# Hanbo-Cheng/DAWN-pytorch

Measured on NVIDIA H100. Metric: denoising-steps/sec (200-frame 256^2 clip), higher is better.
Workload: dtype f32

## Files before the change

dawn_pytorch_b200/_lib.py:

```python
import ctypes
import os

import torch

_HERE = os.path.dirname(os.path.abspath(__file__))
LIB_PATH = os.path.join(_HERE, "libdawn_unet.so")


class DawnUnetCfg(ctypes.Structure):
    _fields_ = [("dim", ctypes.c_int), ("n_levels", ctypes.c_int), ("dim_mults", ctypes.c_int * 8),
                ("channels", ctypes.c_int), ("cond_aud", ctypes.c_int), ("cond_pose", ctypes.c_int),
                ("cond_eye", ctypes.c_int), ("out_grid_dim", ctypes.c_int), ("out_conf_dim", ctypes.c_int),
                ("attn_heads", ctypes.c_int), ("attn_dim_head", ctypes.c_int), ("resnet_groups", ctypes.c_int),
                ("init_kernel_size", ctypes.c_int), ("win_width", ctypes.c_int),
                ("upconv", ctypes.c_int), ("pad_mode", ctypes.c_int), ("no_sla", ctypes.c_int)]


class DawnLfgCfg(ctypes.Structure):
    _fields_ = [("num_channels", ctypes.c_int), ("block_expansion", ctypes.c_int), ("max_features", ctypes.c_int),
                ("num_down_blocks", ctypes.c_int), ("num_bottleneck_blocks", ctypes.c_int), ("skips", ctypes.c_int)]


PATH_MMA_SYNC, PATH_TC_GEMM, PATH_TC_GEMM_PRESPLIT, PATH_TC_CONV3, PATH_TC_CONV3_TMA = range(5)
EPI_PLAIN, EPI_QKV_TEMPORAL, EPI_QKV_SLA, EPI_QKV_MID, EPI_CA_GATE, EPI_GN_APPLY = range(6)


class DawnContractionCase(ctypes.Structure):
    _i, _p = ctypes.c_int, ctypes.c_void_p
    _fields_ = [("path", _i), ("epi", _i),
                ("F", _i), ("IH", _i), ("IW", _i), ("Cin", _i), ("lda", _i),
                ("ntaps", _i), ("dy", _i * 52), ("dx", _i * 52), ("in_stride", _i),
                ("OHs", _i), ("OWs", _i), ("OH", _i), ("OW", _i), ("out_stride", _i), ("oy0", _i), ("ox0", _i),
                ("up2", _i),
                ("perm_pb", _i), ("perm_F", _i), ("perm_in", _i), ("perm_out", _i), ("perm_f_lo", _i), ("perm_f_hi", _i),
                ("P", _i),
                ("N", _i), ("ldb", _i), ("ldo", _i), ("ldr", _i), ("drain", _i), ("ln_inline", _i),
                ("rows_per_batch", _i), ("b_batch_stride", ctypes.c_longlong), ("cpg", _i),
                ("q_post_scale", ctypes.c_float),
                ("A", _p), ("B", _p), ("bias", _p), ("Res", _p), ("Out", _p),
                ("stats", _p), ("rowstats", _p), ("wsum", _p), ("rot", _p),
                ("kq", _p), ("nkq", _p), ("gates", _p),
                ("Y", _p), ("ldy", _i), ("gn_stats", _p), ("gn_w", _p), ("gn_b", _p), ("film", _p), ("gn_count", ctypes.c_double)]


FUSED_TEMPORAL, FUSED_ATTN_TC, FUSED_ATTN_SIMT, FUSED_SLA_CTX, FUSED_SLA_OUT, FUSED_SLA_CTX_UNFUSED, FUSED_CA_WT, \
    FUSED_CA_RSTD, FUSED_GN_HCOND, FUSED_TEMPORAL_MMA_SYNC = range(10)


class DawnFusedCase(ctypes.Structure):
    _i, _p = ctypes.c_int, ctypes.c_void_p
    _fields_ = [("kernel", _i), ("F", _i), ("P", _i), ("C", _i), ("band", _i), ("q_lo", _i), ("q_hi", _i),
                ("nseq", _i), ("L", _i), ("pb", _i), ("seq_base_stride", ctypes.c_longlong), ("elem_stride", ctypes.c_longlong),
                ("ldx", _i), ("ldr", _i), ("ldo", _i), ("ld", _i), ("ldb", _i), ("ldy", _i), ("ldbT", _i),
                ("x", _p), ("res", _p), ("out", _p), ("gamma", _p), ("w_qkv", _p), ("w_out", _p), ("rot", _p), ("bias", _p),
                ("qkv", _p), ("Bf", _p), ("out_bias", _p), ("kq", _p), ("nkq", _p), ("G", _p), ("gates", _p), ("Wt", _p),
                ("T", _p), ("Y", _p), ("out16h", _p), ("out16l", _p),
                ("gn_stats", _p), ("gn_count", ctypes.c_double), ("cpg", _i), ("gn_w", _p), ("gn_b", _p), ("film", _p)]


KERNEL_ROWSTATS, KERNEL_GN_APPLY, KERNEL_COND_TABLES, KERNEL_TIME_MLP, KERNEL_FILM, KERNEL_ROTARY, KERNEL_SPLIT_ROWS, \
    KERNEL_NCF_TO_NHWC, KERNEL_FRAME_INVARIANCE, KERNEL_FEA_SHIFT, KERNEL_MAP_REDUCE, KERNEL_INIT_CONV_X3, KERNEL_HEADS_OUT, \
    KERNEL_DDIM_STEP, KERNEL_DDPM_STEP = range(15)
KERNEL_MAX_DESC = 16


class DawnKernelDesc(ctypes.Structure):
    _i, _p = ctypes.c_int, ctypes.c_void_p
    _fields_ = [("off", _i), ("K", _i), ("co", _i), ("ldbT", _i), ("ca", _i),
                ("mW", _p), ("mB", _p), ("Wkv", _p), ("nkv", _p), ("qs", _p), ("ks", _p), ("Wout", _p), ("gout", _p),
                ("ctx", _p), ("kv", _p), ("kq", _p), ("nkq", _p), ("T", _p), ("G", _p),
                ("W", _p), ("b", _p), ("out", _p), ("n", _i)]


class DawnKernelCase(ctypes.Structure):
    _i, _p, _ll = ctypes.c_int, ctypes.c_void_p, ctypes.c_longlong
    _fields_ = [("kernel", _i), ("M", _i), ("C", _i), ("ld", _i), ("ldy", _i), ("ldr", _i), ("ldo", _i),
                ("F", _i), ("H", _i), ("W", _i), ("P", _i), ("clips", _i),
                ("Cpad", _i), ("c0", _i), ("k", _i), ("skip_if", _i), ("cpg", _i), ("t_stride", _i), ("pos0", _i), ("dim", _i),
                ("ng", _i), ("nc", _i), ("cond_ld", _i), ("ndesc", _i),
                ("n", _ll), ("cstride", _ll), ("clip_stride", _ll), ("count", ctypes.c_double), ("eps", ctypes.c_float),
                ("x", _p), ("y", _p), ("res", _p), ("w", _p), ("b", _p), ("w2", _p), ("b2", _p),
                ("map", _p), ("freqs", _p), ("stats", _p), ("t", _p), ("skip_flag", _p),
                ("out", _p), ("out_hi", _p), ("out_lo", _p), ("flag", _p),
                ("desc", DawnKernelDesc * KERNEL_MAX_DESC),
                ("xs", _p), ("e", _p), ("noise", _p), ("scratch", _p), ("tab", _p), ("t_slot", _p), ("num_t", _i),
                ("replicas", _i), ("coef", ctypes.c_float * 5), ("q", ctypes.c_float)]


LFG_MOTION_PACK, LFG_WARP_BLEND, LFG_AFFINE_RELU, LFG_RESIDUAL_BN_RELU, LFG_RELU_AVGPOOL2, LFG_CHW_TO_HWC, LFG_HWC_TO_CHW, \
    LFG_FINAL_CONV = range(8)


class DawnLfgKernelCase(ctypes.Structure):
    _i, _p = ctypes.c_int, ctypes.c_void_p
    _fields_ = [("kernel", _i), ("F", _i), ("H", _i), ("W", _i), ("h", _i), ("w", _i), ("C", _i), ("Cpad", _i),
# ... 188 lines not shown
```

dawn_pytorch_b200/csrc/contraction.cu:

```cuda
#include <algorithm>
#include <cmath>
#include <cstring>

#include "common.cuh"
#include "contraction.cuh"
#include "kernels.cuh"
#include "tc_gemm.cuh"

namespace dawn {

void HostParams::set(const std::string& name, const float* data, const int64_t* shape, int ndim) {
  HostParam p;
  p.shape.assign(shape, shape + ndim);
  int64_t numel = 1;
  for (int64_t s : p.shape) numel *= s;
  p.data.assign(data, data + numel);
  map[name] = std::move(p);
}

int HostParams::need(const std::string& name, const std::vector<int64_t>& shape, const HostParam** out) const {
  auto it = map.find(name);
  if (it == map.end()) { set_last_error(prefix + "missing parameter: " + name); return -1; }
  const HostParam& p = it->second;
  if (p.shape != shape) {
// ... 234 lines not shown
}

int pack_lfg_up(const HostParams& raw, std::vector<void*>& owner, const std::string& name, int co, int ci, UpConv* u) {
  const HostParam *w, *b;
  DAWN_TRY(raw.need(name + ".conv.weight", {co, ci, 3, 3}, &w));
  DAWN_TRY(raw.need(name + ".conv.bias", {co}, &b));
  std::vector<double> s, t;
  DAWN_TRY(bn_affine(raw, name + ".norm", co, s, t));
  std::vector<float> bias(co);
  for (int n = 0; n < co; ++n) bias[n] = (float)((double)b->data[n] * s[n] + t[n]);
  return pack_up_nearest(owner, w->data.data(), ci, co, s.data(), bias, u);
}

int run_up(const GemmParams& in, const UpConv& u, float* out, int ldo, const std::function<int(const GemmParams&)>& run, int border) {
  if (!border) {
    GemmParams p = in;
    set_weights(p, u.all); set_square_taps(p, 3, 1);
    p.up2 = 1; p.Out = out; p.ldo = ldo;
    if (path_ok(p, EPI_PLAIN, DAWN_PATH_TC_CONV3, 0)) return run(p);
  }
  for (int py = 0; py < 2; ++py)
    for (int px = 0; px < 2; ++px) {
      GemmParams q = in;
      set_weights(q, u.cls[py * 2 + px]);
      q.ntaps = 4;
      for (int ty = 0; ty < 2; ++ty)
        for (int tx = 0; tx < 2; ++tx) {
          q.dy[ty * 2 + tx] = (signed char)(u.off[py][ty] + border); q.dx[ty * 2 + tx] = (signed char)(u.off[px][tx] + border);
        }
      q.OH = 2 * in.OHs; q.OW = 2 * in.OWs; q.out_stride = 2; q.oy0 = py; q.ox0 = px;
      q.Out = out; q.ldo = ldo;
      DAWN_TRY(run(q));
    }
  return 0;
}

namespace {

int refuse(const char* why) {
  set_last_error(std::string("dawn_test_contraction: ") + why);
  return -1;
}

struct Owned {
  std::vector<void*> v;
  ~Owned() { free_all(v); }
};

int test_contraction(const dawn_contraction_case& c, cudaStream_t st) {
  if (c.path < DAWN_PATH_MMA_SYNC || c.path > DAWN_PATH_TC_CONV3_TMA) return refuse("unknown path");
  if (c.epi < EPI_PLAIN || c.epi > EPI_GN_APPLY) return refuse("unknown epilogue");
  if (c.ntaps < 1 || c.ntaps > 52 || c.F < 1 || c.N < 1 || c.ldb < c.N || c.lda < c.Cin) return refuse("bad geometry");
  if (!c.A || !c.B) return refuse("A and B are required");
  if (c.epi == EPI_CA_GATE ? !c.gates : !c.Out) return refuse("no output buffer");

  GemmParams p;
  memset(&p, 0, sizeof(p));
  p.A = c.A; p.lda = c.lda; p.Cin = c.Cin;
  p.up2 = c.up2;
  p.IH = c.IH; p.IW = c.IW; p.OHs = c.OHs; p.OWs = c.OWs; p.in_stride = c.in_stride;
  p.ntaps = c.ntaps;
  for (int t = 0; t < c.ntaps; ++t) { p.dy[t] = (signed char)c.dy[t]; p.dx[t] = (signed char)c.dx[t]; }
  p.M = c.F * c.OHs * c.OWs; p.N = c.N; p.K = c.ntaps * c.Cin;
  p.rows_per_batch = c.rows_per_batch > 0 ? c.rows_per_batch : p.M;
  p.perm_pb = c.perm_pb; p.perm_F = c.perm_F; p.perm_in = c.perm_in; p.perm_out = c.perm_out;
  p.perm_f_lo = c.perm_f_lo; p.perm_f_hi = c.perm_f_hi;
  p.B = c.B; p.ldb = c.ldb; p.b_batch_stride = c.b_batch_stride;
  p.Out = c.Out; p.ldo = c.ldo; p.OH = c.OH; p.OW = c.OW; p.out_stride = c.out_stride; p.oy0 = c.oy0; p.ox0 = c.ox0;
  p.bias = c.bias; p.Res = c.Res; p.ldr = c.ldr;
  p.stats = c.stats; p.cpg = c.cpg; p.clips = 1;
  p.rowstats = c.rowstats; p.ln_inline = c.ln_inline; p.wsum = c.wsum; p.rot = c.rot; p.P = c.P;
  p.q_post_scale = c.q_post_scale;
  p.kq = c.kq; p.nkq = c.nkq; p.gates = c.gates;
  p.Y = c.Y; p.ldy = c.ldy; p.gn_stats = c.gn_stats; p.gn_w = c.gn_w; p.gn_b = c.gn_b; p.film = c.film; p.gn_count = c.gn_count;
  p.drain = c.drain;

  const bool ln = c.epi >= EPI_QKV_TEMPORAL && c.epi <= EPI_CA_GATE;
  if (p.ln_inline && (c.path != DAWN_PATH_TC_GEMM || p.ntaps != 1)) return refuse("inline LayerNorm statistics need the gather-producer wgmma GEMM and one tap");
  if (ln && !p.ln_inline && !p.rowstats) return refuse("LayerNorm epilogue without row statistics");
  if (ln && !p.wsum) return refuse("LayerNorm epilogue without wsum");
  if (c.epi == EPI_PLAIN && p.stats && (p.cpg <= 0 || p.N / p.cpg > 8)) return refuse("GroupNorm statistics need 8 groups");

  Owned own;
  if (c.path != DAWN_PATH_MMA_SYNC) {
    std::vector<float> hB((size_t)p.K * p.ldb);
    DAWN_CUDA_OK(cudaMemcpy(hB.data(), p.B, hB.size() * sizeof(float), cudaMemcpyDeviceToHost));
    PackedWeight w;
    DAWN_TRY(upload_weight(own.v, hB, p.K, p.N, p.ldb, {}, &w));
    set_weights(p, w);
    p.bias = c.bias;
  }
  const bool split = c.path == DAWN_PATH_TC_GEMM_PRESPLIT || c.path == DAWN_PATH_TC_CONV3_TMA;
  const size_t scratch_bytes = split ? (size_t)split_rows(p) * p.Cin * 4 : 0;
  if (!path_ok(p, c.epi, c.path, scratch_bytes)) return refuse("the path does not accept this geometry");
  float* scratch = nullptr;
  if (split) DAWN_TRY(dev_alloc(own.v, scratch_bytes / sizeof(float), &scratch));
  DAWN_TRY(launch_path(p, c.epi, c.path, scratch, st));
  DAWN_CUDA_OK(cudaStreamSynchronize(st));
  return 0;
}

}
}

extern "C" int dawn_test_contraction(const dawn_contraction_case* c, void* stream) {
  if (!c) return dawn::refuse("null case");
  return dawn::test_contraction(*c, static_cast<cudaStream_t>(stream));
}
```

dawn_pytorch_b200/csrc/gemm.cuh:

```cuda
#pragma once
#include <cuda_runtime.h>

namespace dawn {

enum Epi : int {
  EPI_PLAIN = 0,
  EPI_QKV_TEMPORAL = 1,
  EPI_QKV_SLA = 2,
  EPI_QKV_MID = 3,
  EPI_CA_GATE = 4,
  EPI_GN_APPLY = 5,
};

struct GemmParams {
  const float* A; int lda; int Cin;
  const unsigned short* A16h = nullptr; const unsigned short* A16l = nullptr;
  int want_split = 0;
  int up2 = 0;
  int IH, IW;
  int OHs, OWs;
  int in_stride;
  int ntaps; signed char dy[52]; signed char dx[52];
  int M, N, K;
  int rows_per_batch;
  int perm_pb, perm_F, perm_in, perm_out;
  int perm_f_lo, perm_f_hi;
  const float* B; int ldb; long long b_batch_stride;
  const float* Bimg;
  float tc_scale;
  float* Out; int ldo; int OH, OW, out_stride, oy0, ox0;
  const float* bias;
  const float* Res; int ldr;
  double* stats; int cpg;
  int clips;
  const float* rowstats;
  int ln_inline;
  const float* wsum;
  const float* rot;
  int P;
  float q_post_scale;
  const float* kq;
  const float* nkq;
  float* gates;
  const float* Y; int ldy; const double* gn_stats; const float* gn_w; const float* gn_b;
  const float* film;
  double gn_count;
  const int* skip_flag; int skip_if;
  int drain;
};

__host__ __device__ inline int seq_blocked_pixel(int m, int pb, int F, int P) {
  const int blk = m / (F * pb), rem = m - blk * F * pb;
  const int f = rem / pb, pi = rem - f * pb;
  return f * P + blk * pb + pi;
}
__host__ __device__ inline int seq_blocked_out_pixel(int m, int pb, int F, int P, int f_lo, int f_hi) {
  const int blk = m / (F * pb), rem = m - blk * F * pb;
  const int f = rem / pb, pi = rem - f * pb;
  if (f < f_lo || f >= f_hi) return -1;
  return (f - f_lo) * P + blk * pb + pi;
}

int launch_gemm(const GemmParams& p, int epi, cudaStream_t st);

}
```

dawn_pytorch_b200/csrc/tc_conv3.cu:

```cuda
#include <cuda.h>
#include <cuda_fp16.h>
#include <cstdlib>
#include <cstring>
#include <string>
#include <map>
#include <tuple>
#include "common.cuh"
#include "f16x3.cuh"
#include "gemm.cuh"
#include "tc_common.cuh"
#include "tc_gemm.cuh"

namespace dawn {
namespace {

using namespace tc;

constexpr int TH = 16, TW = 8;
constexpr int HH = TH + 2, HW = TW + 2;
constexpr int NPROD = 256;
constexpr int PAIR_HH = 8 + 2;
constexpr int PAIR_ROW_B = 104;

template <int BN, bool PAIR = false>
struct CCfg {
  static_assert(!PAIR || BN == 64, "the pair-mode halos fit next to 64-column weight stages only");
  static constexpr int NWG = BN / 64;
  static constexpr bool SPLIT_EPI = (BN == 64);
  static constexpr int B_PANEL = BN * 128;
  static constexpr int FRAME_ROWS = PAIR ? PAIR_HH * HW : HH * HW;
  static constexpr int HALO_ROWS = PAIR ? PAIR_ROW_B + FRAME_ROWS : FRAME_ROWS;
  static constexpr int A_HALO = (HALO_ROWS * 128 + 1023) / 1024 * 1024;
  static constexpr int A_STAGES = 2;
  static constexpr int B_STAGES = PAIR ? 3 : (BN == 64) ? 4 : 2;
  static constexpr int A_BYTES = A_STAGES * 2 * A_HALO;
  static constexpr int B_BYTES = B_STAGES * 2 * B_PANEL;
  static constexpr int ACC_STAGE = 2 * 128 * kStageLd * 4;
  static constexpr int SMEM_DYN = A_BYTES + B_BYTES + ACC_STAGE + 1024;
  static_assert(SMEM_DYN + 1024 <= 232448, "shared memory");
  static constexpr int EPI_WARP = NPROD / 32 + 4 * NWG;
  static constexpr int LOAD_WARP = EPI_WARP + (SPLIT_EPI ? 4 : 0);
  static constexpr int NTHREADS = 32 * LOAD_WARP + 128;
  static constexpr uint32_t REG_LAUNCH = (65536 / NTHREADS) & ~7u;
  static constexpr uint32_t REG_LOAD = 24, REG_MMA = SPLIT_EPI ? 136 : 128, REG_EPI = 128;
  static_assert(REG_LOAD < REG_LAUNCH && REG_MMA > REG_LAUNCH && REG_EPI > REG_LAUNCH, "register budgets");
  static_assert(2 * REG_LAUNCH + REG_LOAD + NWG * REG_MMA + (SPLIT_EPI ? REG_EPI : 0) <= NTHREADS / 128 * REG_LAUNCH, "CTA register pool");
};

template <int BN, bool TMA, bool PAIR>
__device__ __forceinline__ void tc_conv3_body(const GemmParams& p, const float* __restrict__ Bimg, int tiles_y, int tiles_x, int tiles_n,
                                              int img_bn, const CUtensorMap& tm_hi, const CUtensorMap& tm_lo) {
  using C = CCfg<BN, PAIR>;
  constexpr int B_PANEL = C::B_PANEL, A_STAGES = C::A_STAGES, B_STAGES = C::B_STAGES, NWG = C::NWG;
  constexpr int A_HALO = C::A_HALO, FRAME_ROWS = C::FRAME_ROWS;
  constexpr bool SPLIT = C::SPLIT_EPI;
  extern __shared__ uint8_t smem_raw[];
  __shared__ uint64_t a_full[A_STAGES], a_free[A_STAGES], b_full[B_STAGES], b_free[B_STAGES];
  __shared__ uint64_t st_full[2], st_free[2];
  __shared__ float s_stat[NWG][16];
  __shared__ __align__(16) float s_bias[NWG][64];

  const int tid = threadIdx.x, lane = tid & 31;
  const int warp = __shfl_sync(0xffffffffu, tid >> 5, 0);
  uint8_t* smem = smem_align1024(smem_raw);
  uint8_t* smemA = smem;
  uint8_t* smemB = smem + C::A_BYTES;
  float* stage_base = reinterpret_cast<float*>(smemB + C::B_BYTES);

  if (tid == 0) {
    for (int s = 0; s < A_STAGES; ++s) { mbar_init(&a_full[s], TMA ? 1 : NPROD); mbar_init(&a_free[s], 4 * NWG); }
    for (int s = 0; s < B_STAGES; ++s) { mbar_init(&b_full[s], 1); mbar_init(&b_free[s], 4 * NWG); }
    for (int s = 0; s < 2; ++s) { mbar_init(&st_full[s], 128); mbar_init(&st_free[s], 128); }
    asm volatile("fence.mbarrier_init.release.cluster;" ::: "memory");
  }
  __syncthreads();

  const int H = p.IH, W = p.IW;
  const int F = p.M / (H * W);
  const int NCH = p.Cin / 64;
  const int tiles_sp = tiles_y * tiles_x;
  const int fpc = F / p.clips;
  const int ppc = (fpc + 1) / 2;
  const int total_tiles = (PAIR ? p.clips * ppc : F * tiles_sp) * tiles_n;
  auto decode = [&](int tile, int& f, int& y0, int& x0, int& nt, int& nf) {
    nt = tile % tiles_n;
    const int sp = tile / tiles_n;
    if constexpr (PAIR) {
      const int clip = sp / ppc, fa = 2 * (sp - clip * ppc);
      f = fa * p.clips + clip;
      nf = fa + 1 < fpc ? 2 : 1;
      y0 = 0; x0 = 0;
    } else {
      const int seq = sp / tiles_sp;
      const int r = sp - seq * tiles_sp;
      f = p.clips == 1 ? seq : (seq % fpc) * p.clips + seq / fpc;
      nf = 1;
      y0 = (r / tiles_x) * TH; x0 = (r % tiles_x) * TW;
    }
  };

  if (warp < 8) {
    if (TMA) {
      if (tid == 0) {
        const uint64_t mh = reinterpret_cast<uint64_t>(&tm_hi), ml = reinterpret_cast<uint64_t>(&tm_lo);
        uint32_t ait = 0;
        for (int tile = blockIdx.x; tile < total_tiles; tile += gridDim.x) {
          int f, y0, x0, nt, nf;
          decode(tile, f, y0, x0, nt, nf);
          for (int cc = 0; cc < NCH; ++cc, ++ait) {
            const int s = ait % A_STAGES;
            mbar_wait(&a_free[s], ((ait / A_STAGES) & 1) ^ 1);
            mbar_arrive_expect_tx(&a_full[s], nf * 2 * FRAME_ROWS * 128);
// ... 26 lines not shown
          auto load = [&](int q, float4& a, float4& b) {
            const int l = r0 + 32 * q;
            const int fr = (!PAIR || 32 * q + 31 < FRAME_ROWS) ? 0 : (32 * q >= FRAME_ROWS) ? 1 : (l >= FRAME_ROWS ? 1 : 0);
            const int r = l - fr * FRAME_ROWS;
            const int hy = r / HW, hx = r - hy * HW;
            const int iy = y0 + hy - 1, ix = x0 + hx - 1;
            const bool ok = (r < FRAME_ROWS) && fr < nf && (iy >= 0) && (iy < H) && (ix >= 0) && (ix < W);
            if (ok) {
              const float* fimg = fr ? img_b : img;
              const float4* src = reinterpret_cast<const float4*>(fimg + (size_t)(iy * W + ix) * p.lda + cc * 64) + 2 * c16;
              a = __ldg(src);
              b = __ldg(src + 1);
            } else {
              a = make_float4(0.f, 0.f, 0.f, 0.f);
              b = make_float4(0.f, 0.f, 0.f, 0.f);
            }
          };
          uint8_t* a_hi = smemA + s * 2 * A_HALO;
          uint8_t* a_lo = a_hi + A_HALO;
          auto store = [&](int q, const float4& a, const float4& b) {
            const int lr = r0 + 32 * q;
            const int fr = (!PAIR || 32 * q + 31 < FRAME_ROWS) ? 0 : (32 * q >= FRAME_ROWS) ? 1 : (lr >= FRAME_ROWS ? 1 : 0);
            const int r = lr + fr * (PAIR_ROW_B - FRAME_ROWS);
            if (lr < FRAME_ROWS * (PAIR ? 2 : 1)) {
              uint32_t h[4], l[4];
              split_f16x2_rn(a.x, a.y, h[0], l[0]);
              split_f16x2_rn(a.z, a.w, h[1], l[1]);
              split_f16x2_rn(b.x, b.y, h[2], l[2]);
              split_f16x2_rn(b.z, b.w, h[3], l[3]);
              const uint32_t off = swz(r, c16);
              *reinterpret_cast<uint4*>(a_hi + off) = make_uint4(h[0], h[1], h[2], h[3]);
              *reinterpret_cast<uint4*>(a_lo + off) = make_uint4(l[0], l[1], l[2], l[3]);
            }
          };
          constexpr int NPRE = NQ < 6 ? NQ : 6;
          float4 v[2 * NPRE];
#pragma unroll
          for (int q = 0; q < NPRE; ++q) load(q, v[2 * q], v[2 * q + 1]);
          mbar_wait(&a_free[s], (round & 1) ^ 1);
#pragma unroll
          for (int q = 0; q < NPRE; ++q) store(q, v[2 * q], v[2 * q + 1]);
#pragma unroll
          for (int q = NPRE; q < NQ; ++q) {
            float4 a, b;
            load(q, a, b);
            store(q, a, b);
          }
          mbar_arrive_relaxed(&a_full[s]);
        }
      }
    }
    return;
  }
  if (warp >= C::LOAD_WARP) {
    setmaxnreg_dec<C::REG_LOAD>();
    if (warp == C::LOAD_WARP && lane == 0) {
      uint32_t bit = 0;
      const int KC = 9 * NCH;
      const int sub = PAIR ? img_bn / BN : 1;
      const size_t ipanel = (size_t)sub * B_PANEL;
      for (int tile = blockIdx.x; tile < total_tiles; tile += gridDim.x) {
        int f, y0, x0, nt, nf;
        decode(tile, f, y0, x0, nt, nf);
        const uint8_t* src = reinterpret_cast<const uint8_t*>(Bimg) + (size_t)(nt / sub) * KC * (2 * ipanel) + (size_t)(nt % sub) * B_PANEL;
        for (int cc = 0; cc < NCH; ++cc)
          for (int tap = 0; tap < 9; ++tap, ++bit) {
            const int s = bit % B_STAGES;
            const uint32_t round = bit / B_STAGES;
            mbar_wait(&b_free[s], (round & 1) ^ 1);
            mbar_arrive_expect_tx(&b_full[s], 2 * B_PANEL);
            const uint8_t* panel = src + (size_t)(tap * NCH + cc) * (2 * ipanel);
            if (PAIR) {
              bulk_copy_g2s(smemB + s * 2 * B_PANEL, panel, B_PANEL, &b_full[s]);
              bulk_copy_g2s(smemB + s * 2 * B_PANEL + B_PANEL, panel + ipanel, B_PANEL, &b_full[s]);
            } else {
              bulk_copy_g2s(smemB + s * 2 * B_PANEL, panel, 2 * B_PANEL, &b_full[s]);
            }
          }
      }
    }
    return;
  }

  const int wg = SPLIT ? 0 : (warp - 8) >> 2;
  const int ew = (warp - 8) & 3;
  const int etid = ew * 32 + lane;
  const int bar_id = 2 + wg;
  constexpr uint32_t SBO_HALO = HW * 128;
  constexpr uint32_t H2 = PAIR ? PAIR_ROW_B * 128 : 8 * HW * 128;
  const int dt = (p.drain == 1 || p.drain == 3) ? p.drain : 9;

  auto mma_tile = [&](auto DTc, float* stage, uint32_t& ait, uint32_t& bit, auto&& claim) {
    constexpr int DT = decltype(DTc)::value;
    float d0[32], d1[32];
    bool first_drain = true;
    for (int cc = 0; cc < NCH; ++cc, ++ait) {
      const int sa = ait % A_STAGES;
      mbar_wait(&a_full[sa], (ait / A_STAGES) & 1);
      fence_proxy_async();
      const uint32_t a_hi = smem_u32(smemA + sa * 2 * A_HALO), a_lo = a_hi + A_HALO;
      static_for<0, 9>([&](auto TAPc) {
        constexpr int tap = decltype(TAPc)::value;
        constexpr bool group_first = tap % DT == 0, group_last = tap % DT == DT - 1;
        constexpr uint32_t woff = (uint32_t)(((tap / 3) * HW + tap % 3) * 128);
        const int sb = bit % B_STAGES;
        const int sprev = (bit + B_STAGES - 1) % B_STAGES;
        mbar_wait(&b_full[sb], (bit / B_STAGES) & 1);
        const uint64_t ahi = make_desc(a_hi + woff, SBO_HALO), alo = make_desc(a_lo + woff, SBO_HALO);
        const uint64_t ahi2 = make_desc(a_hi + woff + H2, SBO_HALO), alo2 = make_desc(a_lo + woff + H2, SBO_HALO);
        const uint32_t sbaddr = smem_u32(smemB + sb * 2 * B_PANEL) + wg * 64 * 128;
        const uint64_t bhi = make_desc(sbaddr), blo = make_desc(sbaddr + B_PANEL);
        wgmma_fence();
#pragma unroll
        for (int j = 0; j < 4; ++j) {
          const uint64_t o = (uint64_t)(j * 2);
          const uint32_t acc = (group_first && j == 0) ? 0u : 1u;
          wgmma_m64n64k16(d0, alo + o, bhi + o, acc);
          wgmma_m64n64k16(d1, alo2 + o, bhi + o, acc);
          wgmma_m64n64k16(d0, ahi + o, blo + o, 1u);
          wgmma_m64n64k16(d1, ahi2 + o, blo + o, 1u);
          wgmma_m64n64k16(d0, ahi + o, bhi + o, 1u);
          wgmma_m64n64k16(d1, ahi2 + o, bhi + o, 1u);
        }
        wgmma_commit();
        if constexpr (group_last) {
          wgmma_wait<0>();
          wgmma_fence_acc(d0); wgmma_fence_acc(d1);
          if (lane == 0) { if (!group_first) mbar_arrive(&b_free[sprev]); mbar_arrive(&b_free[sb]); }
          if (first_drain) claim();
          stage_fragment(stage, 0, d0, first_drain, etid);
          stage_fragment(stage, 64, d1, first_drain, etid);
          first_drain = false;
        } else {
          wgmma_wait<1>();
          wgmma_fence_acc(d0); wgmma_fence_acc(d1);
          if (lane == 0 && !group_first) mbar_arrive(&b_free[sprev]);
        }
        ++bit;
      });
      if (lane == 0) mbar_arrive(&a_free[sa]);
    }
  };

  const bool defer_stats = (p.stats != nullptr) && tiles_n == 1;
  const bool bias_smem = (p.bias != nullptr) && tiles_n == 1;
  auto load_bias = [&]() {
    if (bias_smem) {
      if (etid < 64) s_bias[wg][etid] = __ldg(p.bias + wg * 64 + etid);
      asm volatile("bar.sync %0, 128;" ::"r"(bar_id) : "memory");
    }
  };
  auto flush_stats = [&](float (&gs)[8], float (&gss)[8], int clip) {
    const int n0f = wg * 64;
    double* cs = p.stats + 16 * clip;
#pragma unroll
    for (int b8 = 0; b8 < 8; ++b8) {
      double s = (double)gs[b8], ss = (double)gss[b8];
#pragma unroll
      for (int o = 16; o > 0; o >>= 1) { s += __shfl_xor_sync(0xffffffffu, s, o); ss += __shfl_xor_sync(0xffffffffu, ss, o); }
      if (lane == 0) {
        const int grp = (n0f + b8 * 8) / p.cpg;
        atomicAdd(&cs[2 * grp], s);
        atomicAdd(&cs[2 * grp + 1], ss);
      }
      gs[b8] = 0.f; gss[b8] = 0.f;
    }
  };
  auto epilogue_tile = [&](int tile, float* stage, float (&gs)[8], float (&gss)[8], int& pending, int& pclip) {
    int f, y0, x0, nt, nf;
    decode(tile, f, y0, x0, nt, nf);
    const int clip = p.clips > 1 ? f % p.clips : 0;
    const int n0 = nt * BN + wg * 64;
    const int row_in_tile = etid;
    float* s_st = s_stat[wg];
    float* wbuf = stage + ew * 32 * kStageLd;
    float acc[64];
    {
      const float4* src = reinterpret_cast<const float4*>(stage + row_in_tile * kStageLd);
#pragma unroll
      for (int i = 0; i < 16; ++i) {
        const float4 v = src[i];
        acc[4 * i] = v.x; acc[4 * i + 1] = v.y; acc[4 * i + 2] = v.z; acc[4 * i + 3] = v.w;
      }
    }
    __syncwarp();
#pragma unroll
    for (int i = 0; i < 64; ++i) acc[i] *= p.tc_scale;
    const int fr = PAIR ? row_in_tile >> 6 : 0;
    const int img = f + fr * p.clips;
    const int oy = y0 + ((row_in_tile >> 3) & (PAIR ? 7 : 15)), ox = x0 + (row_in_tile & 7);
    const bool rv = (oy < H) && (ox < W) && fr < nf;
    size_t opix = (size_t)img * H * W + (size_t)(rv ? oy * W + ox : 0);
    int ocol = n0;
    if (p.up2) {
      const int cls = n0 >> 6, py = cls >> 1, px = cls & 1;
      opix = (size_t)img * 4 * H * W + (size_t)(rv ? (2 * oy + py) * 2 * W + 2 * ox + px : 0);
      ocol = n0 & 63;
    }
    if (bias_smem) {
      const float4* bp = reinterpret_cast<const float4*>(s_bias[wg]);
#pragma unroll
      for (int i = 0; i < 16; ++i) {
        const float4 b = bp[i];
        acc[4 * i] += b.x; acc[4 * i + 1] += b.y; acc[4 * i + 2] += b.z; acc[4 * i + 3] += b.w;
      }
    } else if (p.bias) {
      const float4* bp = reinterpret_cast<const float4*>(p.bias + n0);
#pragma unroll
      for (int i = 0; i < 16; ++i) {
        const float4 b = __ldg(bp + i);
        acc[4 * i] += b.x; acc[4 * i + 1] += b.y; acc[4 * i + 2] += b.z; acc[4 * i + 3] += b.w;
      }
    }
    store_rows_coalesced(wbuf, acc, p.Out, opix, p.ldo, ocol, rv, lane);
    if (defer_stats) {
      if (pending > 0 && clip != pclip) { flush_stats(gs, gss, pclip); pending = 0; }
      pclip = clip;
      if (rv) {
#pragma unroll
        for (int b8 = 0; b8 < 8; ++b8) {
          float s = 0.f, ss = 0.f;
#pragma unroll
          for (int i = 0; i < 8; ++i) { const float x = acc[b8 * 8 + i]; s += x; ss += x * x; }
          gs[b8] += s; gss[b8] += ss;
        }
      }
      if (++pending == 8) { flush_stats(gs, gss, clip); pending = 0; }
    } else if (p.stats != nullptr) {
      if (etid < 16) s_st[etid] = 0.f;
      asm volatile("bar.sync %0, 128;" ::"r"(bar_id) : "memory");
#pragma unroll
      for (int b8 = 0; b8 < 8; ++b8) {
        float s = 0.f, ss = 0.f;
        if (rv) {
#pragma unroll
          for (int i = 0; i < 8; ++i) { const float x = acc[b8 * 8 + i]; s += x; ss += x * x; }
        }
        s = warp_sum(s); ss = warp_sum(ss);
        if (lane == 0) {
          const int grp = (n0 + b8 * 8) / p.cpg;
          atomicAdd(&s_st[2 * grp], s);
          atomicAdd(&s_st[2 * grp + 1], ss);
        }
      }
      asm volatile("bar.sync %0, 128;" ::"r"(bar_id) : "memory");
      if (etid < 16) {
        const int grp = etid >> 1;
        const int glo = n0 / p.cpg, ghi = (n0 + 63) / p.cpg;
        if (grp >= glo && grp <= ghi) atomicAdd(&p.stats[16 * clip + etid], (double)s_st[etid]);
      }
    }
  };
  auto with_drain = [&](auto&& run) {
    if (dt == 1) run(std::integral_constant<int, 1>{});
    else if (dt == 3) run(std::integral_constant<int, 3>{});
    else run(std::integral_constant<int, 9>{});
  };

  if (SPLIT && warp >= C::EPI_WARP) {
    setmaxnreg_inc<C::REG_EPI>();
    float gs[8], gss[8];
    int pending = 0, pclip = 0;
#pragma unroll
    for (int i = 0; i < 8; ++i) { gs[i] = 0.f; gss[i] = 0.f; }
    load_bias();
    uint32_t lt = 0;
    for (int tile = blockIdx.x; tile < total_tiles; tile += gridDim.x, ++lt) {
      const int b = lt & 1;
      mbar_wait(&st_full[b], (lt >> 1) & 1);
      epilogue_tile(tile, stage_base + b * 128 * kStageLd, gs, gss, pending, pclip);
      mbar_arrive(&st_free[b]);
    }
    if (defer_stats && pending > 0) flush_stats(gs, gss, pclip);
  } else if (SPLIT) {
    setmaxnreg_inc<C::REG_MMA>();
    with_drain([&](auto DTc) {
      uint32_t ait = 0, bit = 0, lt = 0;
      for (int tile = blockIdx.x; tile < total_tiles; tile += gridDim.x, ++lt) {
        const int b = lt & 1;
        mma_tile(DTc, stage_base + b * 128 * kStageLd, ait, bit, [&]() { mbar_wait(&st_free[b], ((lt >> 1) & 1) ^ 1); });
        mbar_arrive(&st_full[b]);
      }
    });
  } else {
    setmaxnreg_inc<C::REG_MMA>();
    float gs[8], gss[8];
    int pending = 0, pclip = 0;
#pragma unroll
    for (int i = 0; i < 8; ++i) { gs[i] = 0.f; gss[i] = 0.f; }
    load_bias();
    float* stage = stage_base + wg * 128 * kStageLd;
    uint32_t ait = 0, bit = 0;
    for (int tile = blockIdx.x; tile < total_tiles; tile += gridDim.x) {
      with_drain([&](auto DTc) { mma_tile(DTc, stage, ait, bit, []() {}); });
      asm volatile("bar.sync %0, 128;" ::"r"(bar_id) : "memory");
      epilogue_tile(tile, stage, gs, gss, pending, pclip);
      asm volatile("bar.sync %0, 128;" ::"r"(bar_id) : "memory");
    }
    if (defer_stats && pending > 0) flush_stats(gs, gss, pclip);
  }
}

template <int BN, bool TMA>
__global__ void __launch_bounds__(CCfg<BN>::NTHREADS, 1) tc_conv3_kernel(const GemmParams p, const float* __restrict__ Bimg,
                                                                          int tiles_y, int tiles_x, int tiles_n, int img_bn,
                                                                          const __grid_constant__ CUtensorMap tm_hi,
                                                                          const __grid_constant__ CUtensorMap tm_lo) {
  tc_conv3_body<BN, TMA, false>(p, Bimg, tiles_y, tiles_x, tiles_n, img_bn, tm_hi, tm_lo);
}

template <bool TMA>
__global__ void __launch_bounds__(CCfg<64, true>::NTHREADS, 1) tc_conv3_pair_kernel(const GemmParams p, const float* __restrict__ Bimg,
                                                                                     int tiles_y, int tiles_x, int tiles_n, int img_bn,
                                                                                     const __grid_constant__ CUtensorMap tm_hi,
                                                                                     const __grid_constant__ CUtensorMap tm_lo) {
  tc_conv3_body<64, TMA, true>(p, Bimg, tiles_y, tiles_x, tiles_n, img_bn, tm_hi, tm_lo);
}

template <int BN, bool TMA, bool PAIR>
constexpr auto c3_kernel() {
  if constexpr (PAIR) return tc_conv3_pair_kernel<TMA>;
  else return tc_conv3_kernel<BN, TMA>;
}

typedef CUresult (*EncodeTiledFn)(CUtensorMap*, CUtensorMapDataType, cuuint32_t, void*, const cuuint64_t*, const cuuint64_t*, const cuuint32_t*,
                                  const cuuint32_t*, CUtensorMapInterleave, CUtensorMapSwizzle, CUtensorMapL2promotion, CUtensorMapFloatOOBfill);
int halo_tensor_map(const void* plane, int Cin, int W, int H, int F, int box_h, CUtensorMap* out) {
  static EncodeTiledFn fn = nullptr;
  if (!fn) {
    void* ptr = nullptr;
    cudaDriverEntryPointQueryResult q;
    DAWN_CUDA_OK(cudaGetDriverEntryPoint("cuTensorMapEncodeTiled", &ptr, cudaEnableDefault, &q));
    if (q != cudaDriverEntryPointSuccess || !ptr) { set_last_error("cuTensorMapEncodeTiled is not available in this driver"); return -2; }
    fn = reinterpret_cast<EncodeTiledFn>(ptr);
  }
  static std::map<std::tuple<const void*, int, int, int, int, int>, CUtensorMap> cache;
  const auto key = std::make_tuple(plane, Cin, W, H, F, box_h);
  auto it = cache.find(key);
  if (it != cache.end()) { *out = it->second; return 0; }
  const cuuint64_t dims[4] = {(cuuint64_t)Cin, (cuuint64_t)W, (cuuint64_t)H, (cuuint64_t)F};
  const cuuint64_t strides[3] = {(cuuint64_t)Cin * 2, (cuuint64_t)W * Cin * 2, (cuuint64_t)H * W * Cin * 2};
  const cuuint32_t box[4] = {64, (cuuint32_t)HW, (cuuint32_t)box_h, 1};
  const cuuint32_t estr[4] = {1, 1, 1, 1};
  CUtensorMap m;
  const CUresult r = fn(&m, CU_TENSOR_MAP_DATA_TYPE_UINT16, 4, const_cast<void*>(plane), dims, strides, box, estr, CU_TENSOR_MAP_INTERLEAVE_NONE,
                        CU_TENSOR_MAP_SWIZZLE_128B, CU_TENSOR_MAP_L2_PROMOTION_L2_128B, CU_TENSOR_MAP_FLOAT_OOB_FILL_NONE);
  if (r != CUDA_SUCCESS) { set_last_error("cuTensorMapEncodeTiled failed with CUresult " + std::to_string((int)r)); return -2; }
  if (cache.size() > 4096) cache.clear();
  cache[key] = m;
  *out = m;
  return 0;
}

template <int BN, bool PAIR>
int launch_c3(const GemmParams& p, const float* Bimg, cudaStream_t st) {
  using C = CCfg<BN, PAIR>;
  static bool attr_set = false;
  static int num_sms = 0;
  if (!attr_set) {
    DAWN_CUDA_OK(cudaFuncSetAttribute(c3_kernel<BN, false, PAIR>(), cudaFuncAttributeMaxDynamicSharedMemorySize, C::SMEM_DYN));
    DAWN_CUDA_OK(cudaFuncSetAttribute(c3_kernel<BN, true, PAIR>(), cudaFuncAttributeMaxDynamicSharedMemorySize, C::SMEM_DYN));
    int dev = 0;
    DAWN_CUDA_OK(cudaGetDevice(&dev));
    DAWN_CUDA_OK(cudaDeviceGetAttribute(&num_sms, cudaDevAttrMultiProcessorCount, dev));
    attr_set = true;
  }
  const int tiles_y = PAIR ? 1 : p.IH / TH, tiles_x = PAIR ? 1 : p.IW / TW, tiles_n = p.N / BN;
  const int F = p.M / (p.IH * p.IW);
  const int seqs = PAIR ? p.clips * ((F / p.clips + 1) / 2) : F;
  const int grid = std::min(seqs * tiles_y * tiles_x * tiles_n, num_sms);
  const int img_bn = tc_tile_n(p.N);
  if (p.A16h != nullptr && p.A16l != nullptr) {
    CUtensorMap mh, ml;
    const int box_h = PAIR ? PAIR_HH : HH;
    if (halo_tensor_map(p.A16h, p.Cin, p.IW, p.IH, F, box_h, &mh) != 0 || halo_tensor_map(p.A16l, p.Cin, p.IW, p.IH, F, box_h, &ml) != 0)
      return -2;
    c3_kernel<BN, true, PAIR>()<<<grid, C::NTHREADS, C::SMEM_DYN, st>>>(p, Bimg, tiles_y, tiles_x, tiles_n, img_bn, mh, ml);
  } else {
    CUtensorMap dummy;
    memset(&dummy, 0, sizeof(dummy));
    c3_kernel<BN, false, PAIR>()<<<grid, C::NTHREADS, C::SMEM_DYN, st>>>(p, Bimg, tiles_y, tiles_x, tiles_n, img_bn, dummy, dummy);
  }
  DAWN_LAUNCH_OK();
  return 0;
}

bool pair_mode(const GemmParams& p) { return p.IH == 8 && p.IW == 8; }

}

bool tc_conv3_supported(const GemmParams& p, int epi) {
  if (epi != EPI_PLAIN || p.Res != nullptr || p.perm_in || p.perm_out) return false;
  if (p.ntaps != 9 || p.in_stride != 1 || p.out_stride != 1 || p.oy0 != 0 || p.ox0 != 0) return false;
  for (int t = 0; t < 9; ++t)
    if (p.dy[t] != t / 3 - 1 || p.dx[t] != t % 3 - 1) return false;
  if (p.IH != p.OH || p.IW != p.OW || p.OHs != p.OH || p.OWs != p.OW) return false;
  if ((p.IH % TH != 0 || p.IW % TW != 0) && !pair_mode(p)) return false;
  if (p.Cin % 64 != 0 || p.N % 64 != 0 || p.K != 9 * p.Cin) return false;
  if (p.b_batch_stride != 0 || p.rows_per_batch != p.M) return false;
  if ((p.lda & 3) || (p.ldo & 3)) return false;
  if (p.stats && (p.cpg % 8 != 0)) return false;
  if (p.up2 && (p.stats != nullptr || p.N != 256)) return false;
  return true;
}

int launch_tc_conv3(const GemmParams& p, const float* Bimg, cudaStream_t st) {
  if (!tc_conv3_supported(p, EPI_PLAIN)) { set_last_error("launch_tc_conv3: unsupported geometry"); return -1; }
  if (pair_mode(p)) return launch_c3<64, true>(p, Bimg, st);
  if (tc_tile_n(p.N) == 128) return launch_c3<128, false>(p, Bimg, st);
  return launch_c3<64, false>(p, Bimg, st);
}

}
```

include/dawn_unet.h:

```cpp
#ifndef DAWN_UNET_H_
#define DAWN_UNET_H_

#include <stdint.h>

#ifdef __cplusplus
extern "C" {
#endif

typedef struct dawn_unet dawn_unet;

typedef struct {
  int dim;
  int n_levels;
  int dim_mults[8];
  int channels;
  int cond_aud;
  int cond_pose;
  int cond_eye;
  int out_grid_dim;
  int out_conf_dim;
  int attn_heads;
  int attn_dim_head;
  int resnet_groups;
  int init_kernel_size;
// ... 39 lines not shown
                   float sigma, float q, void* scratch, void* stream);

int dawn_unet_ddim_step(dawn_unet* h, float* x, const float* eps, const float* noise, int64_t n_local, float ca, float cb,
                        float sqrt_an, float c, float sigma, float q, void* scratch, void* stream);

int dawn_unet_sampler_capture(dawn_unet* h, float* x, float* eps, const float* noise_all, const int64_t* t_all,
                              const float* coef, int nsteps, float q, void* scratch);
int dawn_unet_sampler_launch(dawn_unet* h, void* stream);

int dawn_unet_ddim_step_guided(dawn_unet* h, float* x, const float* eps, const float* noise, int64_t n_clip, const float* cond_scale_dev,
                               float ca, float cb, float sqrt_an, float c, float sigma, float q, void* scratch, void* stream);

int dawn_unet_sampler_capture_guided(dawn_unet* h, float* x, float* eps, const float* noise_all, const int64_t* t_all,
                                     const float* cond_scale_dev, const float* coef, int nsteps, float q, void* scratch);
int dawn_unet_sampler_launch_guided(dawn_unet* h, void* stream);

int dawn_ddpm_step(float* x, const float* eps, const float* noise, int64_t n, float ca, float cb, float c1, float c2,
                   float sigma, float q, void* scratch, void* stream);

int dawn_unet_ddpm_step(dawn_unet* h, float* x, const float* eps, const float* noise, int64_t n_local, float ca, float cb,
                        float c1, float c2, float sigma, float q, void* scratch, void* stream);

int dawn_unet_ddpm_capture(dawn_unet* h, float* x, float* eps, const float* noise, int64_t* t_slot, const float* coef,
                           int num_timesteps, float q, void* scratch);
int dawn_unet_ddpm_launch(dawn_unet* h, void* stream);

enum {
  DAWN_PATH_MMA_SYNC = 0,
  DAWN_PATH_TC_GEMM = 1,
  DAWN_PATH_TC_GEMM_PRESPLIT = 2,
  DAWN_PATH_TC_CONV3 = 3,
  DAWN_PATH_TC_CONV3_TMA = 4
};
typedef struct {
  int path, epi;
  int F, IH, IW, Cin, lda;
  int ntaps; int dy[52]; int dx[52]; int in_stride;
  int OHs, OWs, OH, OW, out_stride, oy0, ox0;
  int up2;
  int perm_pb, perm_F, perm_in, perm_out, perm_f_lo, perm_f_hi;
  int P;
  int N, ldb, ldo, ldr, drain, ln_inline;
  int rows_per_batch;
  long long b_batch_stride;
  int cpg;
  float q_post_scale;
  const float* A; const float* B; const float* bias; const float* Res; float* Out;
  double* stats;
  const float* rowstats;
  const float* wsum;
  const float* rot;
  const float* kq; const float* nkq; float* gates;
  const float* Y; int ldy; const double* gn_stats; const float* gn_w; const float* gn_b; const float* film; double gn_count;
} dawn_contraction_case;
int dawn_test_contraction(const dawn_contraction_case* c, void* stream);

enum {
  DAWN_FUSED_TEMPORAL = 0,
  DAWN_FUSED_ATTN_TC = 1,
  DAWN_FUSED_ATTN_SIMT = 2,
  DAWN_FUSED_SLA_CTX = 3,
  DAWN_FUSED_SLA_OUT = 4,
  DAWN_FUSED_SLA_CTX_UNFUSED = 5,
  DAWN_FUSED_CA_WT = 6,
  DAWN_FUSED_CA_RSTD = 7,
  DAWN_FUSED_GN_HCOND = 8,
  DAWN_FUSED_TEMPORAL_MMA_SYNC = 9
};
typedef struct {
  int kernel;
  int F, P, C;
  int band, q_lo, q_hi;
  int nseq, L, pb;
  long long seq_base_stride, elem_stride;
  int ldx, ldr, ldo, ld, ldb, ldy, ldbT;
  const float* x; const float* res; float* out;
  const float* gamma;
  const float* w_qkv;
  const float* w_out;
  const float* rot;
  const float* bias;
  const float* qkv;
  float* Bf;
  const float* out_bias;
  const float* kq; const float* nkq; const float* G; const float* gates; float* Wt;
  const float* T; const float* Y; unsigned short* out16h; unsigned short* out16l;
  const double* gn_stats; double gn_count; int cpg; const float* gn_w; const float* gn_b; const float* film;
} dawn_fused_case;
int dawn_test_fused(const dawn_fused_case* c, void* stream);

enum {
  DAWN_KERNEL_ROWSTATS = 0,
  DAWN_KERNEL_GN_APPLY = 1,
  DAWN_KERNEL_COND_TABLES = 2,
  DAWN_KERNEL_TIME_MLP = 3,
  DAWN_KERNEL_FILM = 4,
  DAWN_KERNEL_ROTARY = 5,
  DAWN_KERNEL_SPLIT_ROWS = 6,
  DAWN_KERNEL_NCF_TO_NHWC = 7,
  DAWN_KERNEL_FRAME_INVARIANCE = 8,
  DAWN_KERNEL_FEA_SHIFT = 9,
  DAWN_KERNEL_MAP_REDUCE = 10,
  DAWN_KERNEL_INIT_CONV_X3 = 11,
  DAWN_KERNEL_HEADS_OUT = 12,
  DAWN_KERNEL_DDIM_STEP = 13,
  DAWN_KERNEL_DDPM_STEP = 14
// ... 39 lines not shown
```

Baseline: 22.53.

## Use 64-wide column tiles for conv3 and skip zero taps on upsampled inputs

The 3x3 TC conv kernel now defaults to 64-wide output tiles; 128-wide tiles are used only when explicitly requested. For nearest-upsampled inputs with 64-wide tiles, each output parity class needs only 4 distinct input taps (pre-summed weights per class), so the load and MMA loops run 4 taps instead of 9. Bias and GroupNorm stats handling are unified to always use shared-memory bias and deferred stats flushing. The grid is rounded to a multiple of column tiles so each CTA keeps a fixed column class. This depends on the packed weight layout holding per-class combined taps, which this code does not show.

```diff
diff --git a/dawn_pytorch_b200/_lib.py b/dawn_pytorch_b200/_lib.py
--- a/dawn_pytorch_b200/_lib.py
+++ b/dawn_pytorch_b200/_lib.py
@@ -40,7 +40,8 @@
                 ("A", _p), ("B", _p), ("bias", _p), ("Res", _p), ("Out", _p),
                 ("stats", _p), ("rowstats", _p), ("wsum", _p), ("rot", _p),
                 ("kq", _p), ("nkq", _p), ("gates", _p),
-                ("Y", _p), ("ldy", _i), ("gn_stats", _p), ("gn_w", _p), ("gn_b", _p), ("film", _p), ("gn_count", ctypes.c_double)]
+                ("Y", _p), ("ldy", _i), ("gn_stats", _p), ("gn_w", _p), ("gn_b", _p), ("film", _p), ("gn_count", ctypes.c_double),
+                ("clips", _i), ("conv3_bn", _i)]
 
 
 FUSED_TEMPORAL, FUSED_ATTN_TC, FUSED_ATTN_SIMT, FUSED_SLA_CTX, FUSED_SLA_OUT, FUSED_SLA_CTX_UNFUSED, FUSED_CA_WT, \
diff --git a/dawn_pytorch_b200/csrc/contraction.cu b/dawn_pytorch_b200/csrc/contraction.cu
--- a/dawn_pytorch_b200/csrc/contraction.cu
+++ b/dawn_pytorch_b200/csrc/contraction.cu
@@ -310,6 +310,7 @@
   if (c.epi < EPI_PLAIN || c.epi > EPI_GN_APPLY) return refuse("unknown epilogue");
   if (c.ntaps < 1 || c.ntaps > 52 || c.F < 1 || c.N < 1 || c.ldb < c.N || c.lda < c.Cin) return refuse("bad geometry");
   if (!c.A || !c.B) return refuse("A and B are required");
+  if (c.clips > 1 && c.F % c.clips != 0) return refuse("F must be a multiple of clips");
   if (c.epi == EPI_CA_GATE ? !c.gates : !c.Out) return refuse("no output buffer");
 
   GemmParams p;
@@ -326,12 +327,13 @@
   p.B = c.B; p.ldb = c.ldb; p.b_batch_stride = c.b_batch_stride;
   p.Out = c.Out; p.ldo = c.ldo; p.OH = c.OH; p.OW = c.OW; p.out_stride = c.out_stride; p.oy0 = c.oy0; p.ox0 = c.ox0;
   p.bias = c.bias; p.Res = c.Res; p.ldr = c.ldr;
-  p.stats = c.stats; p.cpg = c.cpg; p.clips = 1;
+  p.stats = c.stats; p.cpg = c.cpg; p.clips = c.clips > 1 ? c.clips : 1;
   p.rowstats = c.rowstats; p.ln_inline = c.ln_inline; p.wsum = c.wsum; p.rot = c.rot; p.P = c.P;
   p.q_post_scale = c.q_post_scale;
   p.kq = c.kq; p.nkq = c.nkq; p.gates = c.gates;
   p.Y = c.Y; p.ldy = c.ldy; p.gn_stats = c.gn_stats; p.gn_w = c.gn_w; p.gn_b = c.gn_b; p.film = c.film; p.gn_count = c.gn_count;
   p.drain = c.drain;
+  p.conv3_bn = c.conv3_bn;
 
   const bool ln = c.epi >= EPI_QKV_TEMPORAL && c.epi <= EPI_CA_GATE;
   if (p.ln_inline && (c.path != DAWN_PATH_TC_GEMM || p.ntaps != 1)) return refuse("inline LayerNorm statistics need the gather-producer wgmma GEMM and one tap");
diff --git a/dawn_pytorch_b200/csrc/gemm.cuh b/dawn_pytorch_b200/csrc/gemm.cuh
--- a/dawn_pytorch_b200/csrc/gemm.cuh
+++ b/dawn_pytorch_b200/csrc/gemm.cuh
@@ -47,6 +47,7 @@
   double gn_count;
   const int* skip_flag; int skip_if;
   int drain;
+  int conv3_bn = 0;
 };
 
 __host__ __device__ inline int seq_blocked_pixel(int m, int pb, int F, int P) {
diff --git a/dawn_pytorch_b200/csrc/tc_conv3.cu b/dawn_pytorch_b200/csrc/tc_conv3.cu
--- a/dawn_pytorch_b200/csrc/tc_conv3.cu
+++ b/dawn_pytorch_b200/csrc/tc_conv3.cu
@@ -57,7 +57,6 @@
   extern __shared__ uint8_t smem_raw[];
   __shared__ uint64_t a_full[A_STAGES], a_free[A_STAGES], b_full[B_STAGES], b_free[B_STAGES];
   __shared__ uint64_t st_full[2], st_free[2];
-  __shared__ float s_stat[NWG][16];
   __shared__ __align__(16) float s_bias[NWG][64];
 
   const int tid = threadIdx.x, lane = tid & 31;
@@ -190,25 +189,31 @@
     }
     return;
   }
+  const bool up_taps = BN == 64 && !PAIR && p.up2;
+  const int up_cls = (blockIdx.x % tiles_n) & 3;
+  const int ntaps = up_taps ? 4 : 9;
+  auto tap_of = [&](int t) { return up_taps ? ((up_cls >> 1) + (t >> 1)) * 3 + (up_cls & 1) + (t & 1) : t; };
+
   if (warp >= C::LOAD_WARP) {
     setmaxnreg_dec<C::REG_LOAD>();
     if (warp == C::LOAD_WARP && lane == 0) {
       uint32_t bit = 0;
       const int KC = 9 * NCH;
-      const int sub = PAIR ? img_bn / BN : 1;
+      const int sub = img_bn / BN;
       const size_t ipanel = (size_t)sub * B_PANEL;
       for (int tile = blockIdx.x; tile < total_tiles; tile += gridDim.x) {
         int f, y0, x0, nt, nf;
         decode(tile, f, y0, x0, nt, nf);
         const uint8_t* src = reinterpret_cast<const uint8_t*>(Bimg) + (size_t)(nt / sub) * KC * (2 * ipanel) + (size_t)(nt % sub) * B_PANEL;
         for (int cc = 0; cc < NCH; ++cc)
-          for (int tap = 0; tap < 9; ++tap, ++bit) {
+          for (int t = 0; t < ntaps; ++t, ++bit) {
+            const int tap = tap_of(t);
             const int s = bit % B_STAGES;
             const uint32_t round = bit / B_STAGES;
             mbar_wait(&b_free[s], (round & 1) ^ 1);
             mbar_arrive_expect_tx(&b_full[s], 2 * B_PANEL);
             const uint8_t* panel = src + (size_t)(tap * NCH + cc) * (2 * ipanel);
-            if (PAIR) {
+            if (sub > 1) {
               bulk_copy_g2s(smemB + s * 2 * B_PANEL, panel, B_PANEL, &b_full[s]);
               bulk_copy_g2s(smemB + s * 2 * B_PANEL + B_PANEL, panel + ipanel, B_PANEL, &b_full[s]);
             } else {
@@ -227,9 +232,10 @@
   constexpr uint32_t SBO_HALO = HW * 128;
   constexpr uint32_t H2 = PAIR ? PAIR_ROW_B * 128 : 8 * HW * 128;
   const int dt = (p.drain == 1 || p.drain == 3) ? p.drain : 9;
-
-  auto mma_tile = [&](auto DTc, float* stage, uint32_t& ait, uint32_t& bit, auto&& claim) {
-    constexpr int DT = decltype(DTc)::value;
+  const uint32_t up_woff = (uint32_t)(((up_cls >> 1) * HW + (up_cls & 1)) * 128);
+
+  auto mma_tile = [&](auto DTc, auto NTc, float* stage, uint32_t& ait, uint32_t& bit, auto&& claim) {
+    constexpr int DT = decltype(DTc)::value, NT = decltype(NTc)::value;
     float d0[32], d1[32];
     bool first_drain = true;
     for (int cc = 0; cc < NCH; ++cc, ++ait) {
@@ -237,10 +243,10 @@
       mbar_wait(&a_full[sa], (ait / A_STAGES) & 1);
       fence_proxy_async();
       const uint32_t a_hi = smem_u32(smemA + sa * 2 * A_HALO), a_lo = a_hi + A_HALO;
-      static_for<0, 9>([&](auto TAPc) {
+      static_for<0, NT>([&](auto TAPc) {
         constexpr int tap = decltype(TAPc)::value;
         constexpr bool group_first = tap % DT == 0, group_last = tap % DT == DT - 1;
-        constexpr uint32_t woff = (uint32_t)(((tap / 3) * HW + tap % 3) * 128);
+        const uint32_t woff = NT == 9 ? (uint32_t)(((tap / 3) * HW + tap % 3) * 128) : up_woff + (uint32_t)(((tap / 2) * HW + tap % 2) * 128);
         const int sb = bit % B_STAGES;
         const int sprev = (bit + B_STAGES - 1) % B_STAGES;
         mbar_wait(&b_full[sb], (bit / B_STAGES) & 1);
@@ -280,16 +286,14 @@
     }
   };
 
-  const bool defer_stats = (p.stats != nullptr) && tiles_n == 1;
-  const bool bias_smem = (p.bias != nullptr) && tiles_n == 1;
+  const int n0f = (blockIdx.x % tiles_n) * BN + wg * 64;
   auto load_bias = [&]() {
-    if (bias_smem) {
-      if (etid < 64) s_bias[wg][etid] = __ldg(p.bias + wg * 64 + etid);
+    if (p.bias) {
+      if (etid < 64) s_bias[wg][etid] = __ldg(p.bias + n0f + etid);
       asm volatile("bar.sync %0, 128;" ::"r"(bar_id) : "memory");
     }
   };
   auto flush_stats = [&](float (&gs)[8], float (&gss)[8], int clip) {
-    const int n0f = wg * 64;
     double* cs = p.stats + 16 * clip;
 #pragma unroll
     for (int b8 = 0; b8 < 8; ++b8) {
@@ -310,7 +314,6 @@
     const int clip = p.clips > 1 ? f % p.clips : 0;
     const int n0 = nt * BN + wg * 64;
     const int row_in_tile = etid;
-    float* s_st = s_stat[wg];
     float* wbuf = stage + ew * 32 * kStageLd;
     float acc[64];
     {
@@ -335,23 +338,16 @@
       opix = (size_t)img * 4 * H * W + (size_t)(rv ? (2 * oy + py) * 2 * W + 2 * ox + px : 0);
       ocol = n0 & 63;
     }
-    if (bias_smem) {
+    if (p.bias) {
       const float4* bp = reinterpret_cast<const float4*>(s_bias[wg]);
 #pragma unroll
       for (int i = 0; i < 16; ++i) {
         const float4 b = bp[i];
         acc[4 * i] += b.x; acc[4 * i + 1] += b.y; acc[4 * i + 2] += b.z; acc[4 * i + 3] += b.w;
       }
-    } else if (p.bias) {
-      const float4* bp = reinterpret_cast<const float4*>(p.bias + n0);
-#pragma unroll
-      for (int i = 0; i < 16; ++i) {
-        const float4 b = __ldg(bp + i);
-        acc[4 * i] += b.x; acc[4 * i + 1] += b.y; acc[4 * i + 2] += b.z; acc[4 * i + 3] += b.w;
-      }
     }
     store_rows_coalesced(wbuf, acc, p.Out, opix, p.ldo, ocol, rv, lane);
-    if (defer_stats) {
+    if (p.stats) {
       if (pending > 0 && clip != pclip) { flush_stats(gs, gss, pclip); pending = 0; }
       pclip = clip;
       if (rv) {
@@ -364,35 +360,21 @@
         }
       }
       if (++pending == 8) { flush_stats(gs, gss, clip); pending = 0; }
-    } else if (p.stats != nullptr) {
-      if (etid < 16) s_st[etid] = 0.f;
-      asm volatile("bar.sync %0, 128;" ::"r"(bar_id) : "memory");
-#pragma unroll
-      for (int b8 = 0; b8 < 8; ++b8) {
-        float s = 0.f, ss = 0.f;
-        if (rv) {
-#pragma unroll
-          for (int i = 0; i < 8; ++i) { const float x = acc[b8 * 8 + i]; s += x; ss += x * x; }
-        }
-        s = warp_sum(s); ss = warp_sum(ss);
-        if (lane == 0) {
-          const int grp = (n0 + b8 * 8) / p.cpg;
-          atomicAdd(&s_st[2 * grp], s);
-          atomicAdd(&s_st[2 * grp + 1], ss);
-        }
-      }
-      asm volatile("bar.sync %0, 128;" ::"r"(bar_id) : "memory");
-      if (etid < 16) {
-        const int grp = etid >> 1;
-        const int glo = n0 / p.cpg, ghi = (n0 + 63) / p.cpg;
-        if (grp >= glo && grp <= ghi) atomicAdd(&p.stats[16 * clip + etid], (double)s_st[etid]);
-      }
     }
   };
   auto with_drain = [&](auto&& run) {
-    if (dt == 1) run(std::integral_constant<int, 1>{});
-    else if (dt == 3) run(std::integral_constant<int, 3>{});
-    else run(std::integral_constant<int, 9>{});
+    using I1 = std::integral_constant<int, 1>;
+    if (up_taps) {
+      using I4 = std::integral_constant<int, 4>;
+      if (dt == 1) run(I1{}, I4{});
+      else if (dt == 3) run(std::integral_constant<int, 2>{}, I4{});
+      else run(I4{}, I4{});
+    } else {
+      using I9 = std::integral_constant<int, 9>;
+      if (dt == 1) run(I1{}, I9{});
+      else if (dt == 3) run(std::integral_constant<int, 3>{}, I9{});
+      else run(I9{}, I9{});
+    }
   };
 
   if (SPLIT && warp >= C::EPI_WARP) {
@@ -409,14 +391,14 @@
       epilogue_tile(tile, stage_base + b * 128 * kStageLd, gs, gss, pending, pclip);
       mbar_arrive(&st_free[b]);
     }
-    if (defer_stats && pending > 0) flush_stats(gs, gss, pclip);
+    if (p.stats && pending > 0) flush_stats(gs, gss, pclip);
   } else if (SPLIT) {
     setmaxnreg_inc<C::REG_MMA>();
-    with_drain([&](auto DTc) {
+    with_drain([&](auto DTc, auto NTc) {
       uint32_t ait = 0, bit = 0, lt = 0;
       for (int tile = blockIdx.x; tile < total_tiles; tile += gridDim.x, ++lt) {
         const int b = lt & 1;
-        mma_tile(DTc, stage_base + b * 128 * kStageLd, ait, bit, [&]() { mbar_wait(&st_free[b], ((lt >> 1) & 1) ^ 1); });
+        mma_tile(DTc, NTc, stage_base + b * 128 * kStageLd, ait, bit, [&]() { mbar_wait(&st_free[b], ((lt >> 1) & 1) ^ 1); });
         mbar_arrive(&st_full[b]);
       }
     });
@@ -430,12 +412,12 @@
     float* stage = stage_base + wg * 128 * kStageLd;
     uint32_t ait = 0, bit = 0;
     for (int tile = blockIdx.x; tile < total_tiles; tile += gridDim.x) {
-      with_drain([&](auto DTc) { mma_tile(DTc, stage, ait, bit, []() {}); });
+      with_drain([&](auto DTc, auto NTc) { mma_tile(DTc, NTc, stage, ait, bit, []() {}); });
       asm volatile("bar.sync %0, 128;" ::"r"(bar_id) : "memory");
       epilogue_tile(tile, stage, gs, gss, pending, pclip);
       asm volatile("bar.sync %0, 128;" ::"r"(bar_id) : "memory");
     }
-    if (defer_stats && pending > 0) flush_stats(gs, gss, pclip);
+    if (p.stats && pending > 0) flush_stats(gs, gss, pclip);
   }
 }
 
@@ -506,7 +488,8 @@
   const int tiles_y = PAIR ? 1 : p.IH / TH, tiles_x = PAIR ? 1 : p.IW / TW, tiles_n = p.N / BN;
   const int F = p.M / (p.IH * p.IW);
   const int seqs = PAIR ? p.clips * ((F / p.clips + 1) / 2) : F;
-  const int grid = std::min(seqs * tiles_y * tiles_x * tiles_n, num_sms);
+  if (tiles_n > num_sms) { set_last_error("launch_tc_conv3: more column tiles than SMs"); return -1; }
+  const int grid = std::min(seqs * tiles_y * tiles_x * tiles_n, num_sms / tiles_n * tiles_n);
   const int img_bn = tc_tile_n(p.N);
   if (p.A16h != nullptr && p.A16l != nullptr) {
     CUtensorMap mh, ml;
@@ -539,13 +522,14 @@
   if ((p.lda & 3) || (p.ldo & 3)) return false;
   if (p.stats && (p.cpg % 8 != 0)) return false;
   if (p.up2 && (p.stats != nullptr || p.N != 256)) return false;
+  if (p.conv3_bn != 0 && (p.conv3_bn != 128 || p.N % 128 != 0 || pair_mode(p))) return false;
   return true;
 }
 
 int launch_tc_conv3(const GemmParams& p, const float* Bimg, cudaStream_t st) {
   if (!tc_conv3_supported(p, EPI_PLAIN)) { set_last_error("launch_tc_conv3: unsupported geometry"); return -1; }
   if (pair_mode(p)) return launch_c3<64, true>(p, Bimg, st);
-  if (tc_tile_n(p.N) == 128) return launch_c3<128, false>(p, Bimg, st);
+  if (p.conv3_bn == 128) return launch_c3<128, false>(p, Bimg, st);
   return launch_c3<64, false>(p, Bimg, st);
 }
 
diff --git a/include/dawn_unet.h b/include/dawn_unet.h
--- a/include/dawn_unet.h
+++ b/include/dawn_unet.h
@@ -115,6 +115,8 @@
   const float* rot;
   const float* kq; const float* nkq; float* gates;
   const float* Y; int ldy; const double* gn_stats; const float* gn_w; const float* gn_b; const float* film; double gn_count;
+  int clips;
+  int conv3_bn;
 } dawn_contraction_case;
 int dawn_test_contraction(const dawn_contraction_case* c, void* stream);
 
```

Result: faster. 23.11 (median of 6 runs) (+2.6%).
